# Brown-LEMS/Edge_Based_Visual_Odometry

Measured on AMD Instinct MI355X. Metric: stereo pairs/sec (TOED+NCC match) on KITTI 1241×376; achieved HBM GB/s, higher is better.
Workload: dtype f64; 1 GPU; configs[1]: single KITTI-shaped stereo pair 1241x376 (generator S2, scene 7+rank, 12 px disparity), TOED both images (fp64, no FMA, bit-exact) + epipolar/disparity/orientation candidate search + NCC, resident in HBM, replayed; toed_mode=hybrid, edges_left=126184, edges_right=126340, candidate_pairs=581657, ncc_matches=472947, sims_stored=False, pairs_in_flight_per_gpu=6, streams_per_gpu=4, pairs_submitted_as_hipgraph=2331, toed_strict_fallbacks=0, parallelism=1 independent sequence(s), one per GPU, no collective

## Files before the change

### edge_based_visual_odometry_amd/csrc/ebvo_math.h

```cpp
#ifndef EBVO_MATH_H
#define EBVO_MATH_H

#if defined(__HIPCC__)
#define EBVO_MATH_FN __device__ static inline
#define EBVO_MATH_CONST __device__ __constant__ static const
#else
#define EBVO_MATH_FN static inline
#define EBVO_MATH_CONST static const
#endif

typedef struct
{
    double hi, lo;
} ebvo_dd;

EBVO_MATH_CONST double ebvo_atan_tab[17][2] = {
    {0x0.0p+0, 0x0.0p+0},
    {0x1.ff55bb72cfdeap-5, -0x1.c934d86d23f1dp-60},
    {0x1.fd5ba9aac2f6ep-4, -0x1.cd37686760c17p-59},
    {0x1.7b97b4bce5b02p-3, 0x1.347b0b4f881cap-58},
    {0x1.f5b75f92c80ddp-3, 0x1.8ab6e3cf7afbdp-57},
    {0x1.362773707ebccp-2, -0x1.963a544b672d8p-57},
    {0x1.6f61941e4def1p-2, -0x1.c63aae6f6e918p-56},
    {0x1.a64eec3cc23fdp-2, -0x1.24dec1b50b7ffp-56},
// ... 286 lines not shown

    double f16 = r.hi * 16.0;
    int k = (int)(f16 + (f16 >= 0.0 ? 0.5 : -0.5));
    ebvo_dd u = ebvo_dd_add_d(r, -((double)k * 0.0625));
    int kneg = k < 0;
    int ka = kneg ? -k : k;
    if (ka > 13)
        ka = 13;
    ebvo_dd sk, ck;
    sk.hi = ebvo_sin_tab[ka][0];
    sk.lo = ebvo_sin_tab[ka][1];
    ck.hi = ebvo_cos_tab[ka][0];
    ck.lo = ebvo_cos_tab[ka][1];
    if (kneg)
        sk = ebvo_dd_neg(sk);

    ebvo_dd u2 = ebvo_dd_mul(u, u);
    ebvo_dd u3 = ebvo_dd_mul(u2, u);
    double w = u.hi;
    double z = w * w;
    double ps = 1.0 / 362880.0 - z * (1.0 / 39916800.0);
    ps = 1.0 / 5040.0 - z * ps;
    ps = 1.0 / 120.0 - z * ps;
    ps = ((z * z) * w) * ps;
    ebvo_dd su = ebvo_dd_sub(u, ebvo_dd_div_d(u3, 6.0));
    su = ebvo_dd_add_d(su, ps);
    double pc = 1.0 / 3628800.0 - z * (1.0 / 479001600.0);
    pc = 1.0 / 40320.0 - z * pc;
    pc = 1.0 / 720.0 - z * pc;
    pc = 1.0 / 24.0 - z * pc;
    pc = (z * z) * pc;
    ebvo_dd cu = ebvo_dd_mul_d(u2, -0.5);
    cu = ebvo_dd_add_d(cu, pc);
    cu = ebvo_dd_add_d(cu, 1.0);

    ebvo_dd s = ebvo_dd_add(ebvo_dd_mul(sk, cu), ebvo_dd_mul(ck, su));
    ebvo_dd c = ebvo_dd_sub(ebvo_dd_mul(ck, cu), ebvo_dd_mul(sk, su));
    double sv = s.hi + s.lo, cv = c.hi + c.lo;
    switch (n & 3)
    {
    case 0:
        *sn = sv;
        *cs = cv;
        break;
    case 1:
        *sn = cv;
        *cs = -sv;
        break;
    case 2:
        *sn = -sv;
        *cs = -cv;
        break;
    default:
        *sn = -cv;
        *cs = sv;
        break;
    }
}

EBVO_MATH_FN double ebvo_exp(double x)
{
    if (x != x)
        return x + x;
    if (x > 709.782712893384)
        return 1.7976931348623157e308 * 2.0;
    if (x < -745.2)
        return 0.0;
    double fk = x * EBVO_1_LN2;
    int k = (int)(fk + (fk >= 0.0 ? 0.5 : -0.5));
    double dk = (double)k;
    ebvo_dd r = ebvo_two_sum(x, -(dk * EBVO_LN2_1));
    r = ebvo_dd_add_d(r, -(dk * EBVO_LN2_2));
    ebvo_dd l3;
    l3.hi = EBVO_LN2_3_HI;
    l3.lo = EBVO_LN2_3_LO;
    r = ebvo_dd_sub(r, ebvo_dd_mul_d(l3, dk));
    double f32 = r.hi * 32.0;
    int j = (int)(f32 + (f32 >= 0.0 ? 0.5 : -0.5));
    if (j > 11)
        j = 11;
    if (j < -11)
        j = -11;
    ebvo_dd u = ebvo_dd_add_d(r, -((double)j * 0.03125));
    ebvo_dd u2 = ebvo_dd_mul(u, u);
    ebvo_dd u3 = ebvo_dd_mul(u2, u);
    double w = u.hi;
    double p = 1.0 / 40320.0 + w * (1.0 / 362880.0);
    p = 1.0 / 5040.0 + w * p;
    p = 1.0 / 720.0 + w * p;
    p = 1.0 / 120.0 + w * p;
    p = 1.0 / 24.0 + w * p;
    p = ((w * w) * (w * w)) * p;
    ebvo_dd e = ebvo_dd_add(u, ebvo_dd_mul_d(u2, 0.5));
    e = ebvo_dd_add(e, ebvo_dd_div_d(u3, 6.0));
    e = ebvo_dd_add_d(e, p);
    e = ebvo_dd_add_d(e, 1.0);
    ebvo_dd t;
    t.hi = ebvo_exp_tab[j + 11][0];
    t.lo = ebvo_exp_tab[j + 11][1];
    e = ebvo_dd_mul(t, e);
    double v = e.hi + e.lo;
    return __builtin_ldexp(v, k);
}

EBVO_MATH_FN float ebvo_expf(float x)
{
    if (x != x)
        return x;
    if (x > 88.0f)
        return 3.4028234663852886e38f * 2.0f;
    if (x < -87.0f)
        return 0.0f;
    const float fk = x * 1.44269504088896341f;
    const int k = (int)(fk + (fk >= 0.0f ? 0.5f : -0.5f));
    const float dk = (float)k;
    const float r = (x - dk * 0.693359375f) - dk * -2.12194440e-4f;
    float p = 1.0f / 720.0f;
    p = p * r + 1.0f / 120.0f;
    p = p * r + 1.0f / 24.0f;
    p = p * r + 1.0f / 6.0f;
    p = p * r + 0.5f;
    p = p * r + 1.0f;
    p = p * r + 1.0f;
    return __builtin_ldexpf(p, k);
}

EBVO_MATH_FN float ebvo_fast_atan2_deg(float y, float x)
{
    const float p1 = 0.9997878412794807f * (float)(180 / 3.14159265358979323846);
    const float p3 = -0.3258083974640975f * (float)(180 / 3.14159265358979323846);
    const float p5 = 0.1555786518463281f * (float)(180 / 3.14159265358979323846);
    const float p7 = -0.04432655554792128f * (float)(180 / 3.14159265358979323846);
    const float ax = __builtin_fabsf(x), ay = __builtin_fabsf(y);
    float a, c, c2;
    if (ax >= ay)
    {
        c = ay / (ax + (float)2.2204460492503131e-16);
        c2 = c * c;
        a = (((p7 * c2 + p5) * c2 + p3) * c2 + p1) * c;
    }
    else
    {
        c = ax / (ay + (float)2.2204460492503131e-16);
        c2 = c * c;
        a = 90.f - (((p7 * c2 + p5) * c2 + p3) * c2 + p1) * c;
    }
    if (x < 0)
        a = 180.f - a;
    if (y < 0)
        a = 360.f - a;
    return a;
}

#endif
```

### edge_based_visual_odometry_amd/csrc/match_kernels.hip

```cpp
#include <atomic>
#include <cstdlib>

#include "ebvo_cand.h"
#include "ebvo_internal.h"
#include "ebvo_math.h"

namespace
{

constexpr int BATCH = 64;
constexpr int TILE = 64;
constexpr int STAGE = 64;
struct DevPairs
{
    int64_t host;
    const int32_t *row_ptr;
    DevN nL;
    int64_t cap;
};
__device__ inline int64_t devpairs(const DevPairs &d)
{
    const int64_t n = d.row_ptr ? (int64_t)d.row_ptr[devn(d.nL)] : d.host;
    return n < d.cap ? n : d.cap;
}
// ... 460 lines not shown
            for (int k = (before & ~3) + threadIdx.x; k < before; k += SCAN_BLOCK)
                o += in[k];
        }
        else
            for (int k = threadIdx.x; k < before; k += SCAN_BLOCK)
                o += in[k];
    }
    else
        for (int k = threadIdx.x; k < (int)blockIdx.x; k += SCAN_BLOCK)
            o += S.sums[(size_t)a * S.tiles + k];
    const int32_t tile_off = block_sum_256(o, wpre);
    int32_t v[SCAN_ITEMS];
    int32_t s = 0;
    if (base + SCAN_ITEMS <= n_in && (reinterpret_cast<uintptr_t>(in + base) & 15) == 0)
    {
        const int4 *p = reinterpret_cast<const int4 *>(in + base);
#pragma unroll
        for (int t = 0; t < SCAN_ITEMS / 4; ++t)
        {
            const int4 q = p[t];
            v[4 * t] = q.x; v[4 * t + 1] = q.y; v[4 * t + 2] = q.z; v[4 * t + 3] = q.w;
        }
    }
    else
    {
#pragma unroll
        for (int t = 0; t < SCAN_ITEMS; ++t)
            v[t] = (base + t < n_in) ? in[base + t] : 0;
    }
#pragma unroll
    for (int t = 0; t < SCAN_ITEMS; ++t)
        s += v[t];
    const int lane = threadIdx.x & 63, wid = threadIdx.x >> 6;
    int32_t incl = s;
    for (int d = 1; d < 64; d <<= 1)
    {
        const int32_t t = __shfl_up(incl, d);
        if (lane >= d)
            incl += t;
    }
    if (lane == 63)
        wsum[wid] = incl;
    __syncthreads();
    int32_t pre = 0;
#pragma unroll
    for (int k = 0; k < SCAN_BLOCK / 64; ++k)
        if (k < wid)
            pre += wsum[k];
    int32_t run = tile_off + pre + incl - s;
#pragma unroll
    for (int t = 0; t < SCAN_ITEMS; ++t)
    {
        if (base + t < n)
            out[base + t] = run;
        if (S.n_add == 1 && base + t == n_in && S.total[a])
            *S.total[a] = run;
        run += v[t];
    }
}

__global__ void gather_edges_kernel(const ebvo_edge *__restrict__ R, const int32_t *__restrict__ idx, int64_t n,
                                    ebvo_edge *__restrict__ out)
{
    const int64_t k = (int64_t)blockIdx.x * blockDim.x + threadIdx.x;
    if (k < n)
        out[k] = R[idx[k]];
}

__device__ inline double bilinear_nan(const uint8_t *__restrict__ img, int rows, int cols, int pitch, double x,
                                      double y)
{
    const double x1 = floor(x), x2 = ceil(x);
    const double yc = ceil(y), yf = floor(y);
    const bool inside = (x1 >= 0) && (yf >= 0) && (x2 < cols) && (yc < rows);
    const int c1 = inside ? (int)x1 : 0;
    const int r1 = inside ? (int)yc * pitch : 0, r2 = inside ? (int)yf * pitch : 0;
    unsigned short p1, p2;
    __builtin_memcpy(&p1, img + r1 + c1, 2);
    __builtin_memcpy(&p2, img + r2 + c1, 2);
    const double I11 = (double)(p1 & 0xff);
    const double I21 = (double)(p1 >> 8);
    const double I12 = (double)(p2 & 0xff);
    const double I22 = (double)(p2 >> 8);
    const double wxa = x2 - x;
    const double wxb = x - x1;
    const double wya = -(yf - y);
    const double wyb = -(y - yc);
    const double f1 = wxa * I11 + wxb * I21;
    const double f2 = wxa * I12 + wxb * I22;
    const double v = wya * f1 + wyb * f2;
    const bool ok = inside && (x2 != x1) && (yf != yc);
    return ok ? v : __builtin_nan("");
}

template <int CTRL>
__device__ inline double dpp_f64(double v)
{
    const int lo = __double2loint(v), hi = __double2hiint(v);
    const int plo = __builtin_amdgcn_update_dpp(0, lo, CTRL, 0xf, 0xf, true);
    const int phi = __builtin_amdgcn_update_dpp(0, hi, CTRL, 0xf, 0xf, true);
    return __hiloint2double(phi, plo);
}

__device__ inline double butterfly8(double s)
{
    s += dpp_f64<0xB1>(s);
    s += dpp_f64<0x4E>(s);
    s += dpp_f64<0x141>(s);
    return s;
}

struct PatchBatch
{
    const uint8_t *img[2];
    const ebvo_edge *edges[2];
    DevN n[2];
    double2 *sc[2];
    float *raw[2], *norm[2];
    uint8_t *flag[2];
};

__device__ inline void sincos_body(const ebvo_edge *__restrict__ e, int n, double2 *__restrict__ sc, int vb, int vg)
{
    for (int k = vb * blockDim.x + threadIdx.x; k < n; k += vg * blockDim.x)
    {
        double sn, cs;
        ebvo_sincos(e[k].theta, &sn, &cs);
        double2 v;
        v.x = sn;
        v.y = cs;
        sc[k] = v;
    }
}

__global__ void sincos_batch_kernel(PatchBatch B)
{
    sincos_body(B.edges[blockIdx.y], devn(B.n[blockIdx.y]), B.sc[blockIdx.y], blockIdx.x, gridDim.x);
}

__global__ void sincos_edges_kernel(const ebvo_edge *__restrict__ e, DevN nd, double2 *__restrict__ sc)
{
    const int n = devn(nd);
    for (int k = blockIdx.x * blockDim.x + threadIdx.x; k < n; k += gridDim.x * blockDim.x)
    {
        double sn, cs;
        ebvo_sincos(e[k].theta, &sn, &cs);
        double2 v;
        v.x = sn;
        v.y = cs;
        sc[k] = v;
    }
}

__device__ inline double bilinear_inside_raw(const uint8_t *__restrict__ img, int pitch, double x, double y, bool &ok)
{
    const double wxb = __builtin_amdgcn_fract(x), wya = __builtin_amdgcn_fract(y);
    const double wxa = 1.0 - wxb, wyb = 1.0 - wya;
    const unsigned of = __umul24((unsigned)(int)y, (unsigned)pitch) + (unsigned)(int)x;
    const unsigned oc = of + (unsigned)pitch;
    unsigned short p1, p2;
    __builtin_memcpy(&p1, img + oc, 2);
    __builtin_memcpy(&p2, img + of, 2);
    const double I11 = (double)(p1 & 0xff);
    const double I21 = (double)(p1 >> 8);
    const double I12 = (double)(p2 & 0xff);
    const double I22 = (double)(p2 >> 8);
    const double f1 = wxa * I11 + wxb * I21;
    const double f2 = wxa * I12 + wxb * I22;
    ok = (wxb != 0.0) && (wya != 0.0);
    return wya * f1 + wyb * f2;
}

__device__ inline double bilinear_inside(const uint8_t *__restrict__ img, int pitch, double x, double y)
{
    bool ok;
    const double v = bilinear_inside_raw(img, pitch, x, y, ok);
    return ok ? v : __builtin_nan("");
}

__device__ inline double bilinear_inside2_raw(const uint16_t *__restrict__ pix2, int pitch, double x, double y, bool &ok)
{
    const double wxb = __builtin_amdgcn_fract(x), wya = __builtin_amdgcn_fract(y);
    const double wxa = 1.0 - wxb, wyb = 1.0 - wya;
    const unsigned of = __umul24((unsigned)(int)y, (unsigned)pitch) + (unsigned)(int)x;
    unsigned q;
    __builtin_memcpy(&q, reinterpret_cast<const uint8_t *>(pix2) + 2u * of, 4);
    const double I12 = (double)(q & 0xffu);
    const double I11 = (double)((q >> 8) & 0xffu);
    const double I22 = (double)((q >> 16) & 0xffu);
    const double I21 = (double)(q >> 24);
    const double f1 = wxa * I11 + wxb * I21;
    const double f2 = wxa * I12 + wxb * I22;
    ok = (wxb != 0.0) && (wya != 0.0);
    return wya * f1 + wyb * f2;
}

__device__ inline double bilinear_inside2(const uint16_t *__restrict__ pix2, int pitch, double x, double y)
{
    bool ok;
    const double v = bilinear_inside2_raw(pix2, pitch, x, y, ok);
    return ok ? v : __builtin_nan("");
}

__device__ inline void row_pairs_body(const uint8_t *__restrict__ img, uint16_t *__restrict__ out, int h, int w, int vb, int vg)
{
    const int n = h * w;
    for (int o = (vb * blockDim.x + threadIdx.x) * 4; o < n; o += vg * blockDim.x * 4)
    {
        unsigned a, b = 0;
        __builtin_memcpy(&a, img + o, 4);
        if (o + w + 3 < n)
            __builtin_memcpy(&b, img + o + w, 4);
        else
        {
#pragma unroll
            for (int t = 0; t < 4; ++t)
                if (o + w + t < n)
                    b |= (unsigned)img[o + w + t] << (8 * t);
        }
        uint2 r;
        r.x = (a & 0xffu) | ((b & 0xffu) << 8) | ((a & 0xff00u) << 8) | ((b & 0xff00u) << 16);
        r.y = ((a >> 16) & 0xffu) | (((b >> 16) & 0xffu) << 8) | ((a >> 24) << 16) | ((b >> 24) << 24);
        if (o + 3 < n)
            __builtin_memcpy(out + o, &r, 8);
        else
            for (int t = 0; t < 4 && o + t < n; ++t)
                out[o + t] = (uint16_t)(t < 2 ? (r.x >> (16 * t)) : (r.y >> (16 * (t - 2))));
    }
}

__global__ __launch_bounds__(256) void row_pairs_kernel(const uint8_t *__restrict__ img0, const uint8_t *__restrict__ img1,
                                                        uint16_t *__restrict__ out0, uint16_t *__restrict__ out1, int h,
                                                        int w)
{
    row_pairs_body(blockIdx.y ? img1 : img0, blockIdx.y ? out1 : out0, h, w, blockIdx.x, gridDim.x);
}

struct PrepArgs
{
    const double *F;
    const ebvo_edge *L, *R;
    DevN nL, nR;
    double *lines;
    Box *cb, *gb;
    int32_t *tile_flag;
    int ntiles;
    double2 *scL, *scR;
    const uint8_t *img0, *img1;
    uint16_t *pix0, *pix1;
    int h, w;
    int b_lines, b_boxes, b_sincos, b_rows;
};

__global__ __launch_bounds__(256) void match_prep_kernel(PrepArgs A)
{
    int b = blockIdx.x;
    if (b < A.b_lines)
    {
        lines_body(A.F, A.L, devn(A.nL), A.lines, b, A.b_lines);
        return;
    }
    b -= A.b_lines;
    if (b < A.b_boxes)
    {
        boxes_body(A.R, devn(A.nR), A.cb, A.gb, A.tile_flag, A.ntiles, b, A.b_boxes);
        return;
    }
    b -= A.b_boxes;
    if (b < 2 * A.b_sincos)
    {
        const int im = b >= A.b_sincos;
        sincos_body(im ? A.R : A.L, devn(im ? A.nR : A.nL), im ? A.scR : A.scL, b - im * A.b_sincos, A.b_sincos);
        return;
    }
    b -= 2 * A.b_sincos;
    const int im = b >= A.b_rows;
    row_pairs_body(im ? A.img1 : A.img0, im ? A.pix1 : A.pix0, A.h, A.w, b - im * A.b_rows, A.b_rows);
}

__device__ inline bool patch_inside(int h, int w, double ex, double ey)
{
    return ex >= 9.3 && ey >= 9.3 && ex <= (double)w - 10.3 && ey <= (double)h - 10.3;
}

struct Row7
{
    float v[7];
};

__device__ __noinline__ Row7 sample_row_border(const uint8_t *__restrict__ img, int h, int w, int pitch, double cx, double cy,
                                               double sn, double cs, int i)
{
    Row7 r;
#pragma unroll
    for (int c = 0; c < 7; ++c)
    {
        const int j = c - 3;
        const double x = cs * (i)-sn * (j) + cx;
        const double y = sn * (i) + cs * (j) + cy;
        r.v[c] = (float)bilinear_nan(img, h, w, pitch, x, y);
    }
    return r;
}

template <bool PIX2 = false>
__device__ inline void sample_row(const uint8_t *__restrict__ img, int h, int w, int pitch, double ex, double ey,
                                  double sn, double cs, int side, int row, float p[7], bool active = true,
                                  const uint16_t *__restrict__ pix2 = nullptr )
{
    const double cx = side ? ex + 5 * (-sn) : ex + 5 * (sn);
    const double cy = side ? ey + 5 * (cs) : ey + 5 * (-cs);
    const int i = row - 3;
    if (__all(!active || patch_inside(h, w, ex, ey)))
    {
        bool all_ok = true;
        if (active)
        {
#pragma unroll
            for (int c = 0; c < 7; ++c)
            {
                const int j = c - 3;
                const double x = cs * (i)-sn * (j) + cx;
                const double y = sn * (i) + cs * (j) + cy;
                bool ok;
                p[c] = (float)(PIX2 ? bilinear_inside2_raw(pix2, pitch, x, y, ok) : bilinear_inside_raw(img, pitch, x, y, ok));
                all_ok = all_ok && ok;
            }
        }
        if (__any(!all_ok))
        {
            if (active)
            {
#pragma unroll
                for (int c = 0; c < 7; ++c)
                {
                    const int j = c - 3;
                    const double x = cs * (i)-sn * (j) + cx;
                    const double y = sn * (i) + cs * (j) + cy;
                    if (__builtin_amdgcn_fract(x) == 0.0 || __builtin_amdgcn_fract(y) == 0.0)
                        p[c] = __builtin_nanf("");
                }
            }
        }
        return;
    }
    if (active)
    {
        const Row7 r = sample_row_border(img, h, w, pitch, cx, cy, sn, cs, i);
#pragma unroll
        for (int c = 0; c < 7; ++c)
            p[c] = r.v[c];
    }
}

__device__ inline bool normalise_rows(bool active, const float p[7], float nrm[7])
{
    double rs = 0.0;
    if (active)
    {
        rs = (double)p[0];
#pragma unroll
        for (int c = 1; c < 7; ++c)
            rs += (double)p[c];
    }
    const double mean = butterfly8(rs) / 49.0;
    const float m = (float)mean;
    float d[7];
    double qs = 0.0;
    if (active)
    {
#pragma unroll
        for (int c = 0; c < 7; ++c)
        {
            d[c] = p[c] - m;
            const float q = d[c] * d[c];
            qs = (c == 0) ? (double)q : qs + (double)q;
        }
    }
    const double ss = butterfly8(qs);
    const float inv = (float)(1.0 / sqrt(ss));
#pragma unroll
    for (int c = 0; c < 7; ++c)
        nrm[c] = active ? d[c] * inv : 0.0f;
    return ss < 1e-10;
}

__device__ inline double dot7(const float a[7], const float b[7])
{
    double s = (double)a[0] * (double)b[0];
#pragma unroll
    for (int c = 1; c < 7; ++c)
        s = __builtin_fma((double)a[c], (double)b[c], s);
    return s;
}

__device__ inline double dot_rows(bool active, const float a[7], const float b[7])
{
    return butterfly8(active ? dot7(a, b) : 0.0);
}

__device__ inline double max4(double a, double b, double c, double d)
{
    double m = a;
    if (m < b) m = b;
    if (m < c) m = c;
    if (m < d) m = d;
    return m;
}

__global__ __launch_bounds__(256) void patches_kernel(PatchBatch B, int h, int w, int pitch)
{
    const uint8_t *__restrict__ img = B.img[blockIdx.y];
    const ebvo_edge *__restrict__ edges = B.edges[blockIdx.y];
    const double2 *__restrict__ sc = B.sc[blockIdx.y];
    float *__restrict__ raw = B.raw[blockIdx.y], *__restrict__ norm = B.norm[blockIdx.y];
    uint8_t *__restrict__ flag = B.flag[blockIdx.y];
    const int n = devn(B.n[blockIdx.y]);
    const int groups = (gridDim.x * blockDim.x) >> 4;
    const int t = blockIdx.x * blockDim.x + threadIdx.x;
    const int g = t & 15, side = g >> 3, row = g & 7;
    const int iters = (n + groups - 1) / groups;
    for (int it = 0; it < iters; ++it)
    {
        const int e = it * groups + (t >> 4);
        const bool valid = e < n;
        const bool active = valid && row < 7;
        float p[7], nr[7];
#pragma unroll
        for (int c = 0; c < 7; ++c)
            p[c] = 0.0f;
        {
            const int ec = active ? e : 0;
            sample_row(img, h, w, pitch, edges[ec].x, edges[ec].y, sc[ec].x, sc[ec].y, side, row, p, active);
        }
        const bool sent = normalise_rows(active, p, nr);
        if (active)
        {
            const size_t o = (size_t)e * 98 + side * 49 + row * 7;
            if (raw)
            {
#pragma unroll
                for (int c = 0; c < 7; ++c)
                    raw[o + c] = p[c];
            }
            if (norm)
            {
#pragma unroll
                for (int c = 0; c < 7; ++c)
                    norm[o + c] = nr[c];
            }
            if (flag && row == 0)
                flag[(size_t)e * 2 + side] = sent ? 1 : 0;
        }
    }
}

__global__ __launch_bounds__(256) void ncc_pairs_kernel(const uint8_t *__restrict__ imgR, int h, int w,
                                                        int pitch, const ebvo_edge *__restrict__ Rc,
                                                        const double2 *__restrict__ sc,
                                                        const int32_t *__restrict__ pair_left, DevCount npd,
                                                        const float *__restrict__ left_norm,
                                                        const uint8_t *__restrict__ left_flag, double thr,
                                                        double *__restrict__ sims, double *__restrict__ best,
                                                        uint8_t *__restrict__ keep, int32_t *__restrict__ match_cnt)
{
    const int64_t n_pairs = devcount(npd);
    if ((int64_t)blockIdx.x * 16 >= n_pairs)
        return;
    const int64_t t = (int64_t)blockIdx.x * blockDim.x + threadIdx.x;
    const int64_t k = t >> 4;
    const int g = (int)(t & 15), side = g >> 3, row = g & 7;
    const bool valid = k < n_pairs;
    const bool active = valid && row < 7;
    float p[7], rn[7];
#pragma unroll
    for (int c = 0; c < 7; ++c)
        p[c] = 0.0f;
    int li = 0;
    if (valid)
        li = pair_left[k];
    {
        const int64_t kc = active ? k : 0;
        sample_row(imgR, h, w, pitch, Rc[kc].x, Rc[kc].y, sc[kc].x, sc[kc].y, side, row, p, active);
    }
    const bool rsent = normalise_rows(active, p, rn);
    float lp[7], lm[7];
#pragma unroll
    for (int c = 0; c < 7; ++c)
        lp[c] = lm[c] = 0.0f;
    bool lsent_p = false, lsent_m = false;
    if (active)
// ... 1324 lines not shown
```

### edge_based_visual_odometry_amd/csrc/toed_kernels.hip

```cpp
#include <cstring>

#include <hip/hip_ext.h>

#include "ebvo_internal.h"
#include <atomic>
#include "ebvo_math.h"

namespace
{

const double h_TAP_INT[4][19] = {
    {7.99187055345274e-06, 6.69151128824427e-05, 0.000436341347522880, 0.00221592420596900,
     0.00876415024678427, 0.0269954832565940, 0.0647587978329459, 0.120985362259572, 0.176032663382150,
     0.199471140200716, 0.176032663382150, 0.120985362259572, 0.0647587978329459, 0.0269954832565940,
     0.00876415024678427, 0.00221592420596900, 0.000436341347522880, 6.69151128824427e-05,
     7.99187055345274e-06},
    {1.79817087452687e-05, 0.000133830225764885, 0.000763597358165040, 0.00332388630895351,
     0.0109551878084803, 0.0269954832565940, 0.0485690983747094, 0.0604926811297858, 0.0440081658455374, 0,
     -0.0440081658455374, -0.0604926811297858, -0.0485690983747094, -0.0269954832565940,
     -0.0109551878084803, -0.00332388630895351, -0.000763597358165040, -0.000133830225764885,
     -1.79817087452687e-05},
    {3.84608770384913e-05, 0.000250931673309160, 0.00122721003990810, 0.00443184841193801,
     0.0115029471989044, 0.0202466124424455, 0.0202371243227956, 0, -0.0330061243841531,
     -0.0498677850501791, -0.0330061243841531, 0, 0.0202371243227956, 0.0202466124424455,
// ... 815 lines not shown
    }
    int base_all = pre[0] + pre[1] + pre[2] + pre[3];
    int base_e = pre[(i & 1) * 2], base_o = pre[(i & 1) * 2 + 1];
    int32_t *list_e = lists + (size_t)((i & 1) << 1) * cap;
    const int ncol = W2 - 20;
    for (int c0 = 0; c0 < ncol; c0 += 512)
    {
        const int c = c0 + 8 * lane;
        unsigned mask = 0;
        if (c < ncol)
        {
            unsigned long long x;
            __builtin_memcpy(&x, flag + c, 8);
            const unsigned lo = (unsigned)x, hi = (unsigned)(x >> 32);
            const unsigned tl = ((((lo & 0x7f7f7f7fu) + 0x7f7f7f7fu) | lo) >> 7) & 0x01010101u;
            const unsigned th = ((((hi & 0x7f7f7f7fu) + 0x7f7f7f7fu) | hi) >> 7) & 0x01010101u;
            mask = ((tl * 0x01020408u) >> 24) | (((th * 0x01020408u) >> 24) << 4);
            if (ncol - c < 8)
                mask &= (1u << (ncol - c)) - 1u;
        }
        unsigned total;
        const unsigned front = wave_excl_scan_pair((unsigned)__popc(mask & 0x55u) | ((unsigned)__popc(mask & 0xaau) << 16), total);
        int r_all = base_all + (int)(front & 0xffffu) + (int)(front >> 16);
        int p_e = base_e + (int)(front & 0xffffu), p_o = base_o + (int)(front >> 16);
        const int o0 = i * W2 + 10 + c;
        walk_set_bits(mask, [&](int b) {
            const int par = b & 1;
            if (r_all < cap)
            {
                src[2 * r_all] = o0 + b;
                src[2 * r_all + 1] = -1;
                list_e[(par ? p_o : p_e) + (cap & -par)] = r_all;
            }
            ++r_all;
            p_o += par;
            p_e += par ^ 1;
        });
        base_all += (int)(total & 0xffffu) + (int)(total >> 16);
        base_e += (int)(total & 0xffffu);
        base_o += (int)(total >> 16);
    }
}

struct __attribute__((aligned(64))) CandExact
{
    double gx, gy, m, tox, toy;
    int32_t sector;
    int32_t pad0;
    double pad1[2];
};
static_assert(sizeof(CandExact) == 64, "one cache line per candidate");

__host__ __device__ inline size_t mag_tiles_per_row(int W2) { return (size_t)((W2 + 3) >> 2); }
__host__ __device__ inline size_t mag_map_doubles(int H2, int W2) { return (size_t)((H2 + 1) >> 1) * mag_tiles_per_row(W2) * 8; }
__host__ __device__ inline size_t mag_index(int I, int J, int W2)
{
    return ((size_t)(I >> 1) * mag_tiles_per_row(W2) + (size_t)(J >> 2)) * 8 + (size_t)(((I & 1) << 2) | (J & 3));
}

struct ExactBatch
{
    const uint8_t *img[MAX_BATCH];
    const int32_t *src[MAX_BATCH];
    const int32_t *counts[MAX_BATCH];
    int32_t *lists[MAX_BATCH];
    int32_t *lcount[MAX_BATCH];
    CandExact *cd[MAX_BATCH];
    CandRec *rec[MAX_BATCH];
    int32_t *cand_flag[MAX_BATCH];
    int2 *chunk_cnt[MAX_BATCH];
    const uint8_t *flag[MAX_BATCH];
    uint32_t *needbits[MAX_BATCH];
    int32_t *need_cnt[MAX_BATCH];
    double *magmap[MAX_BATCH];
};

__device__ inline void block_append(bool put, int value, int32_t *__restrict__ list, int32_t *__restrict__ counter,
                                    int *s_cnt )
{
    const int lane = threadIdx.x & 63, wid = threadIdx.x >> 6;
    const unsigned long long m = __ballot(put);
    if (lane == 0)
        s_cnt[wid] = __popcll(m);
    __syncthreads();
    if (threadIdx.x == 0)
    {
        const int tot = s_cnt[0] + s_cnt[1] + s_cnt[2] + s_cnt[3];
        s_cnt[4] = tot ? atomicAdd(counter, tot) : 0;
    }
    __syncthreads();
    if (put)
    {
        int pre = 0;
        for (int k = 0; k < wid; ++k)
            pre += s_cnt[k];
        list[s_cnt[4] + pre + __popcll(m & ((1ull << lane) - 1ull))] = value;
    }
    __syncthreads();
}

struct Row24
{
    unsigned long long w0, w1, w2;
};

__device__ inline Row24 fetch_row(const uint8_t *__restrict__ img, int h, int w, int ii, int j)
{
    const int ic = min(max(ii, 0), h - 1);
    const uint8_t *p = img + (size_t)ic * w + (j - HALO);
    Row24 r;
    __builtin_memcpy(&r.w0, p, 8);
    __builtin_memcpy(&r.w1, p + 8, 8);
    __builtin_memcpy(&r.w2, p + 16, 8);
    return r;
}

struct ColMask
{
    unsigned m[5];
};
__device__ inline ColMask column_mask(int w, int j)
{
    const int lo = max(0, HALO - j), hi = min(19, w + HALO - j);
    ColMask c;
#pragma unroll
    for (int d = 0; d < 5; ++d)
    {
        const int a = min(max(lo - 4 * d, 0), 4), b = min(max(hi - 4 * d, 0), 4);
        const unsigned upto_b = b >= 4 ? 0xffffffffu : ((1u << (8 * b)) - 1u);
        const unsigned upto_a = a >= 4 ? 0xffffffffu : ((1u << (8 * a)) - 1u);
        c.m[d] = upto_b & ~upto_a;
    }
    return c;
}

__device__ inline void mask_row(const Row24 &r, int h, int ii, const ColMask &cm, bool fast, unsigned d[5])
{
    d[0] = (unsigned)r.w0, d[1] = (unsigned)(r.w0 >> 32), d[2] = (unsigned)r.w1, d[3] = (unsigned)(r.w1 >> 32), d[4] = (unsigned)r.w2;
    if (!fast)
    {
        const bool rok = ii >= 0 && ii < h;
#pragma unroll
        for (int k = 0; k < 5; ++k)
            d[k] = rok ? (d[k] & cm.m[k]) : 0u;
    }
}

__device__ inline int row_tap(const unsigned d[5], int q)
{
    const int k = 9 - q;
    return (int)((d[k >> 2] >> (8 * (k & 3))) & 0xffu);
}

__device__ inline void unpack_row(const Row24 &r, int h, int ii, const ColMask &cm, bool fast, int v[19])
{
    unsigned d[5];
    mask_row(r, h, ii, cm, fast, d);
#pragma unroll
    for (int k = 0; k < 19; ++k)
        v[18 - k] = (int)((d[k >> 2] >> (8 * (k & 3))) & 0xffu);
}

__device__ inline bool window_inside(int h, int w, int i, int j)
{
    return i >= HALO && i + HALO < h && j >= HALO && j + HALO < w;
}

constexpr int TAP_K1 = 1000, TAP_K2 = 74;
static_assert(TAP_K1 + TAP_K2 == 1074, "a byte in the low word of a zero register pair is byte * 2^-1074");
struct ExactTaps
{
    double ctap[2][19][4];
    double tap[2][19][4];
    double rtap[2][19][4];
    double prod[17][17][2];
};

__device__ inline double byte_as_subnormal(int b)
{
    return __builtin_bit_cast(double, (unsigned long long)(unsigned)b);
}

__device__ inline void load_exact_taps(ExactTaps &L, const ToedTables *__restrict__ T)
{
    for (int t = threadIdx.x; t < 2 * 19 * 4; t += blockDim.x)
    {
        const int half = t / 76, k = (t % 76) / 4, d = t & 3;
        const double v = half ? T->tap_half[d][k] : T->tap_int[d][k];
        L.tap[half][k][d] = v;
        L.ctap[half][k][d] = ldexp(v, TAP_K1);
        L.rtap[half][k][d] = ldexp(v, TAP_K2);
    }
    for (int t = threadIdx.x; t < 17 * 17; t += blockDim.x)
    {
        const int p = t / 17, q = t % 17;
        L.prod[p][q][0] = T->prod_fx[p][q];
        L.prod[p][q][1] = T->prod_fy[p][q];
    }
    __syncthreads();
}

template <int SY, int SX>
__device__ inline void exact9(const uint8_t *__restrict__ img, int h, int w, const ExactTaps &L, int i, int j,
                              double f[9])
{
    constexpr bool IP = (SY == 0 && SX == 0);
    const double(*ck)[4] = IP ? L.tap[SX] : L.ctap[SX];
    const double(*rk)[4] = IP ? L.tap[SY] : L.rtap[SY];
#pragma unroll
    for (int r = 0; r < 9; ++r)
        f[r] = 0.0;
    constexpr int PM = IP ? 8 : 9;
    const bool fast = __all(window_inside(h, w, i, j));
    const ColMask cm = column_mask(w, j);
    Row24 nxt = fetch_row(img, h, w, i + PM, j);
#pragma unroll 1
    for (int p = -PM; p <= PM; ++p)
    {
        const Row24 cur = nxt;
        nxt = fetch_row(img, h, w, i - min(p + 1, PM), j);
        int vb[19];
        unsigned dw[5];
        if (IP)
            unpack_row(cur, h, i - p, cm, fast, vb);
        else
            mask_row(cur, h, i - p, cm, fast, dw);
        double rr[4];
#pragma unroll
        for (int d = 0; d < 4; ++d)
            rr[d] = rk[p + 9][d];
#pragma unroll
        for (int q = -PM; q <= PM; ++q)
        {
            const double v = IP ? (double)vb[q + 9] : byte_as_subnormal(row_tap(dw, q));
            int lz = 0;
            if (((q + PM) & 3) == 0)
                asm volatile("" : "+v"(lz));
            const double(*ckl)[4] = ck + lz;
            double cc[4];
#pragma unroll
            for (int d = 0; d < 4; ++d)
                cc[d] = v * ckl[q + 9][d];
            if (IP)
            {
                f[0] += v * L.prod[p + 8][q + 8][0];
                f[1] += v * L.prod[p + 8][q + 8][1];
                f[2] += cc[2] * rr[0];
                f[3] += cc[1] * rr[1];
                f[4] += cc[0] * rr[2];
                f[5] += cc[2] * rr[1];
                f[6] += cc[1] * rr[2];
                f[7] += cc[3] * rr[0];
                f[8] += cc[0] * rr[3];
            }
            else
            {
                EBVO_ACCUM9(f, cc, rr)
            }
        }
    }
}

template <int SY, int SX>
__device__ inline double exact_mag(const uint8_t *__restrict__ img, int h, int w, const ExactTaps &L, int I, int J)
{
    constexpr bool IP = (SY == 0 && SX == 0);
    const int i = I >> 1, j = J >> 1;
    const double(*ck)[4] = IP ? L.tap[SX] : L.ctap[SX];
    const double(*rk)[4] = IP ? L.tap[SY] : L.rtap[SY];
    double fx = 0.0, fy = 0.0;
    constexpr int PM = IP ? 8 : 9;
    const bool fast = __all(window_inside(h, w, i, j));
    const ColMask cm = column_mask(w, j);
    Row24 nxt = fetch_row(img, h, w, i + PM, j);
#pragma unroll 1
    for (int p = -PM; p <= PM; ++p)
    {
        const Row24 cur = nxt;
        nxt = fetch_row(img, h, w, i - min(p + 1, PM), j);
        int vb[19];
        unsigned dw[5];
        if (IP)
            unpack_row(cur, h, i - p, cm, fast, vb);
        else
            mask_row(cur, h, i - p, cm, fast, dw);
        const double r0 = rk[p + 9][0], r1 = rk[p + 9][1];
        int lz = 0;
        asm volatile("" : "+v"(lz));
        const double(*ckl)[4] = ck + lz;
#pragma unroll
        for (int q = -PM; q <= PM; ++q)
        {
            const double v = IP ? (double)vb[q + 9] : byte_as_subnormal(row_tap(dw, q));
            if (IP)
            {
                fx += v * L.prod[p + 8][q + 8][0];
                fy += v * L.prod[p + 8][q + 8][1];
            }
            else
            {
                fx += (v * ckl[q + 9][1]) * r0;
                fy += (v * ckl[q + 9][0]) * r1;
            }
        }
    }
    return sqrt(fx * fx + fy * fy);
}

#ifdef EBVO_WAVE_TRACE
__device__ unsigned long long g_wave_trace[2][8192 * 4];
__device__ inline void wave_trace(int which, int wave, unsigned long long t0, int tasks)
{
    if ((threadIdx.x & 63) == 0 && wave < 8192)
    {
        const unsigned hw = __builtin_amdgcn_s_getreg(4 | (0 << 6) | (31 << 11));
        const unsigned xcc = __builtin_amdgcn_s_getreg(20 | (0 << 6) | (31 << 11));
        unsigned long long *o = g_wave_trace[which] + (size_t)wave * 4;
        o[0] = t0;
        o[1] = __builtin_amdgcn_s_memrealtime();
        o[2] = ((unsigned long long)xcc << 32) | hw;
        o[3] = (unsigned long long)tasks;
    }
}
extern "C" int ebvo_wave_trace_read(int which, unsigned long long *dst, int n_waves)
{
    return (int)hipMemcpyFromSymbol(dst, HIP_SYMBOL(g_wave_trace), (size_t)n_waves * 32, (size_t)which * 8192 * 32,
                                    hipMemcpyDeviceToHost);
}
#define EBVO_TRACE_BEGIN() const unsigned long long trace_t0 = __builtin_amdgcn_s_memrealtime(); int trace_n = 0
#define EBVO_TRACE_TASK() ++trace_n
#define EBVO_TRACE_END(which) wave_trace(which, wave, trace_t0, trace_n)
#else
#define EBVO_TRACE_BEGIN()
#define EBVO_TRACE_TASK()
#define EBVO_TRACE_END(which)
#endif

struct ExactTask
{
    int im, ph, k0, n;
};

__device__ inline bool exact_task(const ExactBatch &E, int n_img, int cap, int list0, int t, ExactTask &o)
{
    int base = 0;
    for (int ph = 0; ph < 4; ++ph)
        for (int im = 0; im < n_img; ++im)
        {
            const int n = min(E.lcount[im][list0 + ph], cap);
            const int c = (n + 63) >> 6;
            if (t < base + c)
            {
                o.im = im;
                o.ph = ph;
                o.k0 = (t - base) << 6;
                o.n = n;
                return true;
            }
            base += c;
        }
    return false;
}

template <int SY, int SX>
__device__ inline void centre_run(const ExactBatch &E, const ExactTaps &L, int h, int w, int cap, int im, int k, int n)
{
    const int W2 = 2 * w, H2 = 2 * h, wpr = (W2 + 31) >> 5;
    constexpr int PH = (SY << 1) | SX;
    const int32_t *__restrict__ list = E.lists[im] + (size_t)PH * cap;
    CandExact *__restrict__ cd = E.cd[im];
    const uint8_t *__restrict__ flag = E.flag[im];
    if (k < n)
    {
        const int t = list[k];
        const int o = E.src[im][2 * t];
        const int I = o / W2, J = o - I * W2;
        double f[9];
        exact9<SY, SX>(E.img[im], h, w, L, I >> 1, J >> 1, f);
        const double gx = f[0], gy = f[1];
        const double m = sqrt(gx * gx + gy * gy);
        NmsSector S;
        int packed = -1;
        if (nms_sector(m, gx, gy, S))
        {
            packed = (S.a1 + 1) | ((S.b1 + 1) << 2) | ((S.a2 + 1) << 4) | ((S.b2 + 1) << 6);
#pragma unroll
            for (int q = 0; q < 4; ++q)
            {
                const int da = (q & 2) ? S.a2 : S.a1, db = (q & 2) ? S.b2 : S.b1;
                const int nI = (q & 1) ? I - da : I + da, nJ = (q & 1) ? J - db : J + db;
                const int no = nI * W2 + nJ;
                const bool is_cand = nI >= 10 && nI < H2 - 10 && nJ >= 10 && nJ < W2 - 10 && flag[no] == 1;
                if (!is_cand)
                    atomicOr(&E.needbits[im][(size_t)nI * wpr + (nJ >> 5)], 1u << (nJ & 31));
            }
        }
        CandExact r;
        r.gx = gx;
        r.gy = gy;
        r.m = m;
        third_order_dir(f, r.tox, r.toy);
        r.sector = packed;
        r.pad0 = 0;
        r.pad1[0] = r.pad1[1] = 0.0;
        cd[t] = r;
        E.magmap[im][mag_index(I, J, W2)] = m;
    }
}

#ifndef EBVO_CENTRE_WPS
#define EBVO_CENTRE_WPS 0
#endif
#if EBVO_CENTRE_WPS > 0
__global__ __launch_bounds__(256, EBVO_CENTRE_WPS) void toed_exact_centre_kernel(ExactBatch E, const ToedTables *__restrict__ T, int h,
#else
__global__ __launch_bounds__(256) void toed_exact_centre_kernel(ExactBatch E, const ToedTables *__restrict__ T, int h,
#endif
                                                                int w, int cap, int n_img)
{
    __shared__ ExactTaps L;
    EBVO_TRACE_BEGIN();
    load_exact_taps(L, T);
    const int lane = threadIdx.x & 63;
    const int wave = __builtin_amdgcn_readfirstlane((int)(blockIdx.x * 4 + (threadIdx.x >> 6)));
    ExactTask q;
    for (int t = wave; exact_task(E, n_img, cap, 0, t, q); t += gridDim.x * 4)
    {
        EBVO_TRACE_TASK();
        switch (q.ph)
        {
        case 0: centre_run<0, 0>(E, L, h, w, cap, q.im, q.k0 + lane, q.n); break;
        case 1: centre_run<0, 1>(E, L, h, w, cap, q.im, q.k0 + lane, q.n); break;
        case 2: centre_run<1, 0>(E, L, h, w, cap, q.im, q.k0 + lane, q.n); break;
        default: centre_run<1, 1>(E, L, h, w, cap, q.im, q.k0 + lane, q.n); break;
        }
    }
    EBVO_TRACE_END(0);
}

__global__ __launch_bounds__(256) void toed_need_count_kernel(ExactBatch E, int h, int w)
{
    const int W2 = 2 * w, H2 = 2 * h, wpr = (W2 + 31) >> 5;
    const int im = blockIdx.y, I = blockIdx.x * 4 + (threadIdx.x >> 6), lane = threadIdx.x & 63;
    if (I >= H2)
        return;
    const uint32_t *__restrict__ row = E.needbits[im] + (size_t)I * wpr;
    int ne = 0, no = 0;
    for (int k = lane; k < wpr; k += 64)
    {
        const uint32_t v = row[k];
        ne += __popc(v & 0x55555555u);
        no += __popc(v & 0xaaaaaaaau);
    }
    for (int d = 32; d > 0; d >>= 1)
    {
        ne += __shfl_down(ne, d);
        no += __shfl_down(no, d);
// ... 539 lines not shown
```

Baseline: 3654 stereo pairs/s.

## Replace int-to-double conversions with subnormal bit-cast scaling in bilinear and TOED taps

Replaces integer-to-double conversions of pixel bytes with a bit-cast of each byte into a subnormal double, with weights pre-scaled by powers of two so the products come out exact. Applies this to the NCC bilinear sampling, which also now detects fract==0 through an integer min over the high words instead of compares, and to the in-phase TOED tap loops, which use a prescaled product table with a final unscale. This removes cvt instructions and the separate unpack path and shrinks the LDS tap table. The catch is reliance on subnormal arithmetic being preserved exactly (no denormal flushing) and on asm ordering hints to keep loads in flight.

```diff
diff --git a/edge_based_visual_odometry_amd/csrc/ebvo_math.h b/edge_based_visual_odometry_amd/csrc/ebvo_math.h
--- a/edge_based_visual_odometry_amd/csrc/ebvo_math.h
+++ b/edge_based_visual_odometry_amd/csrc/ebvo_math.h
@@ -462,4 +462,11 @@
     return a;
 }
 
+#if defined(__HIPCC__)
+__device__ inline double byte_as_subnormal(int b)
+{
+    return __builtin_bit_cast(double, (unsigned long long)(unsigned)b);
+}
 #endif
+
+#endif
diff --git a/edge_based_visual_odometry_amd/csrc/match_kernels.hip b/edge_based_visual_odometry_amd/csrc/match_kernels.hip
--- a/edge_based_visual_odometry_amd/csrc/match_kernels.hip
+++ b/edge_based_visual_odometry_amd/csrc/match_kernels.hip
@@ -636,54 +636,71 @@
     }
 }
 
-__device__ inline double bilinear_inside_raw(const uint8_t *__restrict__ img, int pitch, double x, double y, bool &ok)
-{
-    const double wxb = __builtin_amdgcn_fract(x), wya = __builtin_amdgcn_fract(y);
-    const double wxa = 1.0 - wxb, wyb = 1.0 - wya;
+constexpr int SAMPLE_KX = 1000, SAMPLE_KY = 74;
+static_assert(SAMPLE_KX + SAMPLE_KY == 1074, "a byte in the low word of a zero register pair is byte * 2^-1074");
+constexpr double SAMPLE_2KX = 0x1p1000, SAMPLE_2KY = 0x1p74;
+
+__device__ inline unsigned high_word(double v)
+{
+    return (unsigned)(__builtin_bit_cast(unsigned long long, v) >> 32);
+}
+
+constexpr int SAMPLES_IN_FLIGHT = 5;
+struct CornerChain
+{
+    unsigned zero_hi;
+    double last;
+};
+__device__ inline CornerChain corner_chain(double any)
+{
+    CornerChain c;
+    c.zero_hi = 0u;
+    asm("" : "+v"(c.zero_hi));
+    c.last = any;
+    return c;
+}
+template <int S>
+__device__ inline double corner_product(double w, unsigned &q, CornerChain &ch)
+{
+    asm("" : "+v"(q) : "v"(ch.last));
+    const unsigned b = S == 0 ? q & 0xffu : S == 24 ? q >> 24 : __builtin_amdgcn_ubfe(q, S, 8);
+    const unsigned long long pr = ((unsigned long long)ch.zero_hi << 32) | b;
+    ch.last = w * __builtin_bit_cast(double, pr);
+    return ch.last;
+}
+
+template <int S11, int S21, int S12, int S22>
+__device__ inline double bilinear_corners(double x, double y, unsigned q, CornerChain &ch, unsigned &zacc)
+{
+    const double fx = __builtin_amdgcn_fract(x), fy = __builtin_amdgcn_fract(y);
+    zacc = min(min(zacc, high_word(fx)), high_word(fy));
+    const double wxb = fx * SAMPLE_2KX, wya = fy * SAMPLE_2KY;
+    const double wxa = SAMPLE_2KX - wxb, wyb = SAMPLE_2KY - wya;
+    const double a11 = corner_product<S11>(wxa, q, ch), b21 = corner_product<S21>(wxb, q, ch);
+    const double a12 = corner_product<S12>(wxa, q, ch), b22 = corner_product<S22>(wxb, q, ch);
+    const double f1 = a11 + b21;
+    const double f2 = a12 + b22;
+    return wya * f1 + wyb * f2;
+}
+
+__device__ inline double bilinear_inside_raw(const uint8_t *__restrict__ img, int pitch, double x, double y, CornerChain &ch,
+                                             unsigned &zacc)
+{
     const unsigned of = __umul24((unsigned)(int)y, (unsigned)pitch) + (unsigned)(int)x;
     const unsigned oc = of + (unsigned)pitch;
     unsigned short p1, p2;
     __builtin_memcpy(&p1, img + oc, 2);
     __builtin_memcpy(&p2, img + of, 2);
-    const double I11 = (double)(p1 & 0xff);
-    const double I21 = (double)(p1 >> 8);
-    const double I12 = (double)(p2 & 0xff);
-    const double I22 = (double)(p2 >> 8);
-    const double f1 = wxa * I11 + wxb * I21;
-    const double f2 = wxa * I12 + wxb * I22;
-    ok = (wxb != 0.0) && (wya != 0.0);
-    return wya * f1 + wyb * f2;
-}
-
-__device__ inline double bilinear_inside(const uint8_t *__restrict__ img, int pitch, double x, double y)
-{
-    bool ok;
-    const double v = bilinear_inside_raw(img, pitch, x, y, ok);
-    return ok ? v : __builtin_nan("");
-}
-
-__device__ inline double bilinear_inside2_raw(const uint16_t *__restrict__ pix2, int pitch, double x, double y, bool &ok)
-{
-    const double wxb = __builtin_amdgcn_fract(x), wya = __builtin_amdgcn_fract(y);
-    const double wxa = 1.0 - wxb, wyb = 1.0 - wya;
+    return bilinear_corners<16, 24, 0, 8>(x, y, (unsigned)p2 | ((unsigned)p1 << 16), ch, zacc);
+}
+
+__device__ inline double bilinear_inside2_raw(const uint16_t *__restrict__ pix2, int pitch, double x, double y, CornerChain &ch,
+                                              unsigned &zacc)
+{
     const unsigned of = __umul24((unsigned)(int)y, (unsigned)pitch) + (unsigned)(int)x;
     unsigned q;
     __builtin_memcpy(&q, reinterpret_cast<const uint8_t *>(pix2) + 2u * of, 4);
-    const double I12 = (double)(q & 0xffu);
-    const double I11 = (double)((q >> 8) & 0xffu);
-    const double I22 = (double)((q >> 16) & 0xffu);
-    const double I21 = (double)(q >> 24);
-    const double f1 = wxa * I11 + wxb * I21;
-    const double f2 = wxa * I12 + wxb * I22;
-    ok = (wxb != 0.0) && (wya != 0.0);
-    return wya * f1 + wyb * f2;
-}
-
-__device__ inline double bilinear_inside2(const uint16_t *__restrict__ pix2, int pitch, double x, double y)
-{
-    bool ok;
-    const double v = bilinear_inside2_raw(pix2, pitch, x, y, ok);
-    return ok ? v : __builtin_nan("");
+    return bilinear_corners<8, 24, 0, 16>(x, y, q, ch, zacc);
 }
 
 __device__ inline void row_pairs_body(const uint8_t *__restrict__ img, uint16_t *__restrict__ out, int h, int w, int vb, int vg)
@@ -797,21 +814,24 @@
     const int i = row - 3;
     if (__all(!active || patch_inside(h, w, ex, ey)))
     {
-        bool all_ok = true;
+        unsigned zacc = ~0u;
         if (active)
         {
+            CornerChain ch = corner_chain(cx);
+            double done[7];
 #pragma unroll
             for (int c = 0; c < 7; ++c)
             {
                 const int j = c - 3;
-                const double x = cs * (i)-sn * (j) + cx;
-                const double y = sn * (i) + cs * (j) + cy;
-                bool ok;
-                p[c] = (float)(PIX2 ? bilinear_inside2_raw(pix2, pitch, x, y, ok) : bilinear_inside_raw(img, pitch, x, y, ok));
-                all_ok = all_ok && ok;
+                double x = j ? cs * (i)-sn * (j) + cx : cs * (i) + cx;
+                const double y = j ? sn * (i) + cs * (j) + cy : sn * (i) + cy;
+                if (c >= SAMPLES_IN_FLIGHT)
+                    asm("" : "+v"(x) : "v"(done[c - SAMPLES_IN_FLIGHT]));
+                p[c] = (float)(PIX2 ? bilinear_inside2_raw(pix2, pitch, x, y, ch, zacc) : bilinear_inside_raw(img, pitch, x, y, ch, zacc));
+                done[c] = ch.last;
             }
         }
-        if (__any(!all_ok))
+        if (__any(zacc == 0u))
         {
             if (active)
             {
@@ -819,8 +839,8 @@
                 for (int c = 0; c < 7; ++c)
                 {
                     const int j = c - 3;
-                    const double x = cs * (i)-sn * (j) + cx;
-                    const double y = sn * (i) + cs * (j) + cy;
+                    const double x = j ? cs * (i)-sn * (j) + cx : cs * (i) + cx;
+                    const double y = j ? sn * (i) + cs * (j) + cy : sn * (i) + cy;
                     if (__builtin_amdgcn_fract(x) == 0.0 || __builtin_amdgcn_fract(y) == 0.0)
                         p[c] = __builtin_nanf("");
                 }
diff --git a/edge_based_visual_odometry_amd/csrc/toed_kernels.hip b/edge_based_visual_odometry_amd/csrc/toed_kernels.hip
--- a/edge_based_visual_odometry_amd/csrc/toed_kernels.hip
+++ b/edge_based_visual_odometry_amd/csrc/toed_kernels.hip
@@ -991,15 +991,6 @@
     return (int)((d[k >> 2] >> (8 * (k & 3))) & 0xffu);
 }
 
-__device__ inline void unpack_row(const Row24 &r, int h, int ii, const ColMask &cm, bool fast, int v[19])
-{
-    unsigned d[5];
-    mask_row(r, h, ii, cm, fast, d);
-#pragma unroll
-    for (int k = 0; k < 19; ++k)
-        v[18 - k] = (int)((d[k >> 2] >> (8 * (k & 3))) & 0xffu);
-}
-
 __device__ inline bool window_inside(int h, int w, int i, int j)
 {
     return i >= HALO && i + HALO < h && j >= HALO && j + HALO < w;
@@ -1007,18 +998,15 @@
 
 constexpr int TAP_K1 = 1000, TAP_K2 = 74;
 static_assert(TAP_K1 + TAP_K2 == 1074, "a byte in the low word of a zero register pair is byte * 2^-1074");
+constexpr int PROD_KP = 1023;
+constexpr double PROD_UNSCALE = 0x1p51;
+static_assert(1074 - PROD_KP == 51, "PROD_UNSCALE undoes the scale of sprod and of the subnormal byte");
 struct ExactTaps
 {
     double ctap[2][19][4];
-    double tap[2][19][4];
     double rtap[2][19][4];
-    double prod[17][17][2];
+    double sprod[17][17][2];
 };
-
-__device__ inline double byte_as_subnormal(int b)
-{
-    return __builtin_bit_cast(double, (unsigned long long)(unsigned)b);
-}
 
 __device__ inline void load_exact_taps(ExactTaps &L, const ToedTables *__restrict__ T)
 {
@@ -1026,15 +1014,14 @@
     {
         const int half = t / 76, k = (t % 76) / 4, d = t & 3;
         const double v = half ? T->tap_half[d][k] : T->tap_int[d][k];
-        L.tap[half][k][d] = v;
         L.ctap[half][k][d] = ldexp(v, TAP_K1);
         L.rtap[half][k][d] = ldexp(v, TAP_K2);
     }
     for (int t = threadIdx.x; t < 17 * 17; t += blockDim.x)
     {
         const int p = t / 17, q = t % 17;
-        L.prod[p][q][0] = T->prod_fx[p][q];
-        L.prod[p][q][1] = T->prod_fy[p][q];
+        L.sprod[p][q][0] = ldexp(T->prod_fx[p][q], PROD_KP);
+        L.sprod[p][q][1] = ldexp(T->prod_fy[p][q], PROD_KP);
     }
     __syncthreads();
 }
@@ -1044,8 +1031,8 @@
                               double f[9])
 {
     constexpr bool IP = (SY == 0 && SX == 0);
-    const double(*ck)[4] = IP ? L.tap[SX] : L.ctap[SX];
-    const double(*rk)[4] = IP ? L.tap[SY] : L.rtap[SY];
+    const double(*ck)[4] = L.ctap[SX];
+    const double(*rk)[4] = L.rtap[SY];
 #pragma unroll
     for (int r = 0; r < 9; ++r)
         f[r] = 0.0;
@@ -1058,12 +1045,8 @@
     {
         const Row24 cur = nxt;
         nxt = fetch_row(img, h, w, i - min(p + 1, PM), j);
-        int vb[19];
         unsigned dw[5];
-        if (IP)
-            unpack_row(cur, h, i - p, cm, fast, vb);
-        else
-            mask_row(cur, h, i - p, cm, fast, dw);
+        mask_row(cur, h, i - p, cm, fast, dw);
         double rr[4];
 #pragma unroll
         for (int d = 0; d < 4; ++d)
@@ -1071,7 +1054,7 @@
 #pragma unroll
         for (int q = -PM; q <= PM; ++q)
         {
-            const double v = IP ? (double)vb[q + 9] : byte_as_subnormal(row_tap(dw, q));
+            const double v = byte_as_subnormal(row_tap(dw, q));
             int lz = 0;
             if (((q + PM) & 3) == 0)
                 asm volatile("" : "+v"(lz));
@@ -1082,8 +1065,8 @@
                 cc[d] = v * ckl[q + 9][d];
             if (IP)
             {
-                f[0] += v * L.prod[p + 8][q + 8][0];
-                f[1] += v * L.prod[p + 8][q + 8][1];
+                f[0] += v * L.sprod[p + 8][q + 8][0];
+                f[1] += v * L.sprod[p + 8][q + 8][1];
                 f[2] += cc[2] * rr[0];
                 f[3] += cc[1] * rr[1];
                 f[4] += cc[0] * rr[2];
@@ -1098,6 +1081,11 @@
             }
         }
     }
+    if (IP)
+    {
+        f[0] *= PROD_UNSCALE;
+        f[1] *= PROD_UNSCALE;
+    }
 }
 
 template <int SY, int SX>
@@ -1105,8 +1093,8 @@
 {
     constexpr bool IP = (SY == 0 && SX == 0);
     const int i = I >> 1, j = J >> 1;
-    const double(*ck)[4] = IP ? L.tap[SX] : L.ctap[SX];
-    const double(*rk)[4] = IP ? L.tap[SY] : L.rtap[SY];
+    const double(*ck)[4] = L.ctap[SX];
+    const double(*rk)[4] = L.rtap[SY];
     double fx = 0.0, fy = 0.0;
     constexpr int PM = IP ? 8 : 9;
     const bool fast = __all(window_inside(h, w, i, j));
@@ -1117,12 +1105,8 @@
     {
         const Row24 cur = nxt;
         nxt = fetch_row(img, h, w, i - min(p + 1, PM), j);
-        int vb[19];
         unsigned dw[5];
-        if (IP)
-            unpack_row(cur, h, i - p, cm, fast, vb);
-        else
-            mask_row(cur, h, i - p, cm, fast, dw);
+        mask_row(cur, h, i - p, cm, fast, dw);
         const double r0 = rk[p + 9][0], r1 = rk[p + 9][1];
         int lz = 0;
         asm volatile("" : "+v"(lz));
@@ -1130,11 +1114,11 @@
 #pragma unroll
         for (int q = -PM; q <= PM; ++q)
         {
-            const double v = IP ? (double)vb[q + 9] : byte_as_subnormal(row_tap(dw, q));
+            const double v = byte_as_subnormal(row_tap(dw, q));
             if (IP)
             {
-                fx += v * L.prod[p + 8][q + 8][0];
-                fy += v * L.prod[p + 8][q + 8][1];
+                fx += v * L.sprod[p + 8][q + 8][0];
+                fy += v * L.sprod[p + 8][q + 8][1];
             }
             else
             {
@@ -1142,6 +1126,11 @@
                 fy += (v * ckl[q + 9][0]) * r1;
             }
         }
+    }
+    if (IP)
+    {
+        fx *= PROD_UNSCALE;
+        fy *= PROD_UNSCALE;
     }
     return sqrt(fx * fx + fy * fy);
 }
```

New measurement: 3680 stereo pairs/s, median of 6. Within noise of the previous version (+0.7%).
